# r-barnes/richdem

Measured on NVIDIA H100. Metric: Priority-Flood fill + D8 flow accumulation throughput, higher is better.
Workload: dtype f32

## Files before the change

richdem_b200/csrc/capi.cu:

```cuda
#include "common.cuh"

#include <algorithm>
#include <cstdlib>
#include <type_traits>

namespace rdb {

static thread_local std::string g_last_error;

void capi_set_error(const char *msg) { g_last_error = msg ? msg : "unknown error"; }

Ctx &ctx() {
  static Ctx c;
  return c;
}

static void init_device(int device) {
  Ctx &c = ctx();
  if (c.inited && c.device == device) return;
  if (c.inited) fail("rdb200_init: already initialised on device %d (call rdb200_shutdown first)", c.device);
  int ndev = 0;
  cudaError_t e = cudaGetDeviceCount(&ndev);
  if (e != cudaSuccess || ndev == 0)
    fail("no CUDA device available (%s); librichdem_b200 has no CPU fallback",
// ... 1 lines not shown
  if (device < 0 || device >= ndev) fail("rdb200_init: device %d out of range (0..%d)", device, ndev - 1);
  RDB_CK(cudaSetDevice(device));
  cudaDeviceProp prop;
  RDB_CK(cudaGetDeviceProperties(&prop, device));
  if (prop.major != 9 || prop.minor != 0)
    fail("device %d is sm_%d%d; librichdem_b200 is built for sm_90a (H100) only", device, prop.major,
         prop.minor);
  c.device = device;
  c.num_sms = prop.multiProcessorCount;
  RDB_CK(cudaStreamCreate(&c.own_stream));
  c.stream = c.own_stream;
  RDB_CK(cudaEventCreate(&c.ev0));
  RDB_CK(cudaEventCreate(&c.ev1));
  RDB_CK(cudaEventCreate(&c.evk0));
  RDB_CK(cudaEventCreate(&c.evk1));
  c.pinned_bytes = 1 << 16;
  RDB_CK(cudaMallocHost(&c.pinned, c.pinned_bytes));
  memset(&c.stats, 0, sizeof(c.stats));
  c.inited = true;
}

void ensure_init() {
  Ctx &c = ctx();
  if (c.inited) {
    RDB_CK(cudaSetDevice(c.device));
    return;
  }
  int dev = 0;
  cudaError_t e = cudaGetDevice(&dev);
  if (e != cudaSuccess) dev = 0;
// ... 394 lines not shown
int rdb200_init(int device) {
  return capi_call([&] { init_device(device); });
}

void rdb200_shutdown(void) {
  Ctx &c = ctx();
  if (!c.inited) return;
  cudaSetDevice(c.device);
  cudaStreamSynchronize(c.stream);
  ws_release_all();
  if (c.pinned) cudaFreeHost(c.pinned);
  cudaEventDestroy(c.ev0);
  cudaEventDestroy(c.ev1);
  cudaEventDestroy(c.evk0);
  cudaEventDestroy(c.evk1);
  cudaStreamDestroy(c.own_stream);
  for (int k = 0; k < 2; k++)
    if (c.aux_stream[k]) cudaStreamDestroy(c.aux_stream[k]);
  for (int k = 0; k < 3; k++)
    if (c.aux_event[k]) cudaEventDestroy(c.aux_event[k]);
  const Params keep = c.params;
  c = Ctx();
  c.params = keep;
}

const char *rdb200_last_error(void) { return g_last_error.c_str(); }
int rdb200_version(void) { return RDB200_VERSION; }

int rdb200_set_stream(void *cuda_stream) {
  return capi_call([&] {
// ... 31 lines not shown
    else if (n == "fill_wake_filter") p.fill_wake_filter = value;
    else if (n == "fill_trace") p.fill_trace = value;
    else if (n == "fill_ordered") p.fill_ordered = value;
    else if (n == "fill_order_rounds") p.fill_order_rounds = value;
    else if (n == "fill_band_rounds") p.fill_band_rounds = value;
    else if (n == "accum_threads") p.accum_threads = value > 0 ? value : 256;
    else if (n == "accum_budget") p.accum_budget = value;
    else if (n == "accum_walk_lanes") p.accum_walk_lanes = value;
    else if (n == "accum_fused_prep") p.accum_fused_prep = value;
    else if (n == "flats_tiled") p.flats_tiled = value;
    else if (n == "flats_pair") p.flats_pair = value;
    else if (n == "flats_fused_classify") p.flats_fused_classify = value;
    else if (n == "fill_multigrid") p.fill_multigrid = value;
    else if (n == "fill_multigrid_min") p.fill_multigrid_min = value;
    else if (n == "fill_vcycle") p.fill_vcycle = value;
    else if (n == "fill_band_multigrid") p.fill_band_multigrid = value;
    else if (n == "flats_uf_tiled") p.flats_uf_tiled = value;
    else if (n == "flowdirs_rolling") p.flowdirs_rolling = value;
    else if (n == "accum_packed") p.accum_packed = value;
    else if (n == "accum_dinf_packed") p.accum_dinf_packed = value;
    else if (n == "accum_dinf_share") p.accum_dinf_share = value;
    else if (n == "flowmet_tarboton_filter") p.flowmet_tarboton_filter = value;
    else if (n == "accum_walk_scan") p.accum_walk_scan = value;
    else if (n == "accum_walk_ahead") p.accum_walk_ahead = value;
    else if (n == "accum_dinf_stats") p.accum_dinf_stats = value;
    else if (n == "accum_dinf_wait") p.accum_dinf_wait = value;
    else if (n == "f64_band_rank_cap") p.f64_band_rank_cap = value;
    else fail("rdb200_set_param: unknown parameter '%s'", name);
  });
}
// ... 426 lines not shown
```

richdem_b200/csrc/common.cuh:

```cuda
#pragma once

#include <cuda.h>
#include <cuda_runtime.h>

#include <cstdarg>
#include <cstdint>
#include <cstdio>
#include <cstring>
#include <stdexcept>
#include <string>
#include <vector>

#include "../../include/richdem_b200.h"

struct rdb200_fill_state;

namespace rdb {

struct Error : std::runtime_error {
  using std::runtime_error::runtime_error;
};

[[noreturn]] inline void fail(const char *fmt, ...) {
  char buf[1024];
// ... 34 lines not shown
}

struct Params {
  int64_t fill_max_iters = 0;
  int64_t fill_rounds_per_sync = 16;
  int64_t fill_use_tma = 1;
  int64_t fill_external_z = 1;
  int64_t fill_ordered = 1;
  int64_t fill_order_rounds = 0;
  int64_t fill_band_rounds = 0;
  int64_t fill_profile = 0;
  int64_t fill_wake_filter = 1;
  int64_t fill_trace = 0;
  int64_t fill_multigrid = 8;
  int64_t fill_vcycle = 8;
  int64_t fill_band_multigrid = 0;
  int64_t fill_multigrid_min = 0;
  int64_t flowdirs_rolling = 1;
  int64_t flats_uf_tiled = 1;
  int64_t flats_fused_classify = 1;
  int64_t flats_pair = 1;
  int64_t flats_tiled = 1;
  int64_t accum_dinf_packed = 1;
  int64_t flowmet_tarboton_filter = 1;
  int64_t accum_walk_ahead = 0;
  int64_t accum_walk_scan = 0;
  int64_t accum_dinf_stats = 0;
  int64_t accum_dinf_share = -1;
  int64_t accum_dinf_wait = 0;
  int64_t accum_packed = 1;
// ... 4 lines not shown
  int64_t f64_band_rank_cap = 0;
};

struct WsBlock {
  void *ptr;
  size_t bytes;
  bool in_use;
};

struct Ctx {
  bool inited = false;
  int device = -1;
  int num_sms = 0;
  cudaStream_t stream = nullptr;
  cudaStream_t own_stream = nullptr;
  cudaEvent_t ev0 = nullptr, ev1 = nullptr, evk0 = nullptr, evk1 = nullptr;
  cudaStream_t aux_stream[2] = {nullptr, nullptr};
  cudaEvent_t aux_event[3] = {nullptr, nullptr, nullptr};
  std::vector<WsBlock> ws;
  void *pinned = nullptr;
  size_t pinned_bytes = 0;
  rdb200_stats stats;
  Params params;
};

Ctx &ctx();
void ensure_init();
void *ws_alloc(size_t bytes);
void ws_free(void *p);
void ws_release_all();

// ... 140 lines not shown
```

richdem_b200/csrc/fill.cu:

```cuda
#include "common.cuh"

#include <chrono>
#include <memory>

namespace rdb {

namespace {

#ifndef RDB_TX
#define RDB_TX 64
#endif
#ifndef RDB_TY
#define RDB_TY 64
#endif
#ifndef RDB_FILL_THREADS
#define RDB_FILL_THREADS 128
#endif
#ifndef RDB_FILL_MIN_CTAS
#define RDB_FILL_MIN_CTAS 6
#endif
constexpr int TX = RDB_TX;
constexpr int TY = RDB_TY;
constexpr int BXN = TX / 4;
constexpr int BYN = TY / 4;
// ... 16 lines not shown
  RoundCtl proc[3];
  unsigned long long visits;
  unsigned long long iters;
  unsigned long long block_updates;
  unsigned long long warp_updates;
  unsigned long long idle_visits;
  unsigned long long wakes_dropped;
  unsigned long long iter_hist[8];
  int edge_changed;
  int zmin_ord, zmax_ord;
  unsigned long long deferred;
  unsigned long long live_rounds;
  float level, step, step_min, level_max;
  int target, ordered;
  int ndefer[3];
};

struct FillArgs {
  const float *Z;
  int zpitch, zox, zoy;
  int inplace;
  const float *coarse;
  int Wc, pool, yoff;
  int *staged;
  float *zcopy;
  float *Wp;
  int pitch;
  int wox, woy;
  int W, H;
  int tilesX, tilesY;
  int *list0, *list1;
  int *stamp;
  int *sides;
  int *keys;
  float level;
  int *plist;
  int use_proc;
  FillDev *dev;
  int round;
  int max_iters;
  int use_tma;
  int profile;
  int *dirty;
  unsigned long long *edge_above;
};

__device__ __forceinline__ uint32_t smem_u32(const void *p) {
  return (uint32_t)__cvta_generic_to_shared(p);
}
__device__ __forceinline__ void mbar_init(unsigned long long *bar, int count) {
  asm volatile("mbarrier.init.shared::cta.b64 [%0], %1;" ::"r"(smem_u32(bar)), "r"(count) : "memory");
}
__device__ __forceinline__ void mbar_arrive_expect_tx(unsigned long long *bar, uint32_t bytes) {
  asm volatile("mbarrier.arrive.expect_tx.shared::cta.b64 _, [%0], %1;" ::"r"(smem_u32(bar)),
               "r"(bytes)
               : "memory");
}
__device__ __forceinline__ void mbar_wait(unsigned long long *bar, uint32_t parity) {
// ... 47 lines not shown
  const int b = o >= 0 ? o : (o ^ 0x7fffffff);
  float f;
  memcpy(&f, &b, 4);
  return f;
}
constexpr int ORD_POS_INF = 0x7f800000;

__device__ __forceinline__ void enqueue_tile(const FillArgs &a, RoundCtl *next, int *list_next, int t,
                                             int stampval, int side_bits, int key_ord) {
  atomicOr(&a.sides[(stampval & 1) * a.tilesX * a.tilesY + t], side_bits);
  atomicMin(&a.keys[(stampval & 1) * a.tilesX * a.tilesY + t], key_ord);
  if (atomicExch(&a.stamp[t], stampval) != stampval) {
    const int idx = atomicAdd(&next->count, 1);
    list_next[idx] = t;
  }
}

__device__ __forceinline__ float min3f(float a, float b, float c) { return fminf(fminf(a, b), c); }

__host__ __device__ __forceinline__ float next_up(float x) {
  int b;
  memcpy(&b, &x, 4);
  b = b < 0 ? (b == (int)0x80000000 ? 1 : b - 1) : (b < 0x7f800000 ? b + 1 : b);
  float r;
  memcpy(&r, &b, 4);
  return r;
}

template <int STEP>
__device__ __forceinline__ float fill_step(float w) {
// ... 319 lines not shown
                   *reinterpret_cast<const float4 *>(&sZ[rr * TX + 4 * cc]));
        }
      }
    }
    if (stage) {
      __syncthreads();
      if (tid == 0) {
        __threadfence();
        atomicExch(&a.staged[t], 1);
      }
    }
    if (STEP != 1 && WAKE_WORDS && a.edge_above) {
      fill_wake_neighbours<TOPO4>(a, sW, sZ, t, fl, sKey, next, list_next);
      if (rowch && tid == 0) {
        if (fl & (3 << 9)) atomicOr(&a.dev->edge_changed, (fl >> 9) & 3);
        if (a.dirty) a.dirty[t] = 1;
      }
    } else if (rowch) {
      if (tid < 8) {
        const int sv = r + 1;
        const bool n_ok = tyT > 0, s_ok = tyT < a.tilesY - 1, w_ok = txT > 0, e_ok = txT < a.tilesX - 1;
        int nb = -1, bits = 0;
        switch (tid) {
          case 0: if ((fl & SIDE_N) && n_ok) { nb = t - a.tilesX; bits = SIDE_S; } break;
          case 1: if ((fl & SIDE_S) && s_ok) { nb = t + a.tilesX; bits = SIDE_N; } break;
          case 2: if ((fl & SIDE_W) && w_ok) { nb = t - 1; bits = SIDE_E; } break;
          case 3: if ((fl & SIDE_E) && e_ok) { nb = t + 1; bits = SIDE_W; } break;
          case 4: if ((fl & SIDE_NW) && n_ok && w_ok) { nb = t - a.tilesX - 1; bits = SIDE_SE; } break;
          case 5: if ((fl & SIDE_NE) && n_ok && e_ok) { nb = t - a.tilesX + 1; bits = SIDE_SW; } break;
          case 6: if ((fl & SIDE_SW) && s_ok && w_ok) { nb = t + a.tilesX - 1; bits = SIDE_NE; } break;
          default: if ((fl & SIDE_SE) && s_ok && e_ok) { nb = t + a.tilesX + 1; bits = SIDE_NW; } break;
        }
        if (nb >= 0) enqueue_tile(a, next, list_next, nb, sv, bits, sKey);
        if (tid == 0 && (fl & (3 << 9))) atomicOr(&a.dev->edge_changed, (fl >> 9) & 3);
        if (tid == 0 && a.dirty) a.dirty[t] = 1;
      }
    }
    if (tid == 0) {
      if (again) enqueue_tile(a, next, list_next, t, r + 1, SIDE_FULL, f2ord(-__int_as_float(0x7f800000)));
      atomicAdd(&a.dev->iters, (unsigned long long)iters);
      if (a.profile) {
        if (!rowch) atomicAdd(&a.dev->idle_visits, 1ull);
        atomicAdd(&a.dev->block_updates, (unsigned long long)sProf[0]);
        atomicAdd(&a.dev->warp_updates, (unsigned long long)sProf[1]);
        const int hb = iters <= 1 ? 0 : iters <= 2 ? 1 : iters <= 4 ? 2 : iters <= 8 ? 3 : iters <= 16 ? 4 : iters <= 32 ? 5 : iters <= 64 ? 6 : 7;
        atomicAdd(&a.dev->iter_hist[hb], 1ull);
      }
    }
  }
  if (STAGE && a.use_tma && tid == 0) bulk_wait_all();
// ... 16 lines not shown
    if (ord2f(kord) <= level) {
      a.plist[atomicAdd(&proc->count, 1)] = t;
    } else {
      int bits = a.sides[(r & 1) * ntiles + t];
      if (bits == 0) bits = SIDE_FULL;
      a.sides[(r & 1) * ntiles + t] = 0;
      a.keys[(r & 1) * ntiles + t] = ORD_POS_INF;
      enqueue_tile(a, next, list_next, t, r + 1, bits, kord);
      nd++;
    }
  }
  for (int o = 16; o > 0; o >>= 1) nd += __shfl_xor_sync(0xffffffffu, nd, o);
  if ((threadIdx.x & 31) == 0 && nd) atomicAdd(&a.dev->ndefer[r % 3], nd);
}

__global__ void __launch_bounds__(256) fill_seed_kernel(const FillArgs a, const int *__restrict__ tiles, int n) {
  const int i = blockIdx.x * blockDim.x + threadIdx.x;
  if (i >= n) return;
  const int r = a.round;
  RoundCtl *cur = &a.dev->ctl[r % 3];
  int *list_cur = (r & 1) ? a.list1 : a.list0;
  enqueue_tile(a, cur, list_cur, tiles[i], r, SIDE_FULL, f2ord(-__int_as_float(0x7f800000)));
}

__global__ void __launch_bounds__(256) fill_seed_flags_kernel(const FillArgs a, const int *__restrict__ flag, int ntiles,
                                                               int *count) {
  const int t = blockIdx.x * blockDim.x + threadIdx.x;
  if (t >= ntiles || !flag[t]) return;
  const int r = a.round;
  RoundCtl *cur = &a.dev->ctl[r % 3];
  int *list_cur = (r & 1) ? a.list1 : a.list0;
  enqueue_tile(a, cur, list_cur, t, r, SIDE_FULL, f2ord(-__int_as_float(0x7f800000)));
  if (count) atomicAdd(count, 1);
}

__global__ void __launch_bounds__(256) fill_ghost_update_kernel(float *Wp, float *Zp, int pitch, int W, int H, int y,
                                                                 const float *__restrict__ row, int *tile_flag, int tilesX,
                                                                 int *lowered) {
// ... 189 lines not shown
    }
    float *o = Wc + (size_t)(by + coy) * cpitch + bx + cox;
    if (m < *o && bx > 0 && by > 0 && bx < Wcw - 1 && by < Hc - 1) {
      *o = m;
      const int ty0 = (by - 1) / TY, ty1 = (by + 1) / TY, tx0 = (bx - 1) / TX, tx1 = (bx + 1) / TX;
      ctile_flag[ty0 * ctilesX + tx0] = 1;
      if (tx1 != tx0) ctile_flag[ty0 * ctilesX + tx1] = 1;
      if (ty1 != ty0) {
        ctile_flag[ty1 * ctilesX + tx0] = 1;
        if (tx1 != tx0) ctile_flag[ty1 * ctilesX + tx1] = 1;
      }
    }
  }
}

__global__ void __launch_bounds__(256) fill_blockmax_kernel(const float *__restrict__ Wp, int pitch, int wox, int woy, int W,
                                                             int y_lo, int y_hi,
                                                             int yoff, float *out, int Wcw, int Hc, int k,
                                                             const int *__restrict__ dirty, int tilesX) {
  const int bx = blockIdx.x * blockDim.x + threadIdx.x;
  if (bx >= Wcw) return;
  const int by_lo = (yoff + y_lo) / k, by_hi = (yoff + y_hi - 1) / k;
  for (int by = by_lo + blockIdx.y; by <= by_hi && by < Hc; by += gridDim.y) {
    if (dirty) {
      int l0 = by * k - yoff, l1 = l0 + k - 1;
      l0 = l0 < y_lo ? y_lo : l0;
      l1 = l1 >= y_hi ? y_hi - 1 : l1;
      const int tx = (bx * k) / TX;
      if (!dirty[(l0 / TY) * tilesX + tx] && !dirty[(l1 / TY) * tilesX + tx]) {
        out[(size_t)by * Wcw + bx] = __int_as_float(0x7f800000);
// ... 3 lines not shown
    float m = -__int_as_float(0x7f800000);
    for (int j = 0; j < k; j++) {
      const int y = by * k + j - yoff;
      if (y < y_lo) continue;
      if (y >= y_hi) break;
      for (int i = 0; i < k; i++) {
        const int x = bx * k + i;
        if (x < W) m = fmaxf(m, __ldcg(Wp + (size_t)(y + woy) * pitch + x + wox));
      }
    }
    float *o = out + (size_t)by * Wcw + bx;
    *o = fmaxf(*o, m);
  }
}

__global__ void __launch_bounds__(256) fill_prolong_kernel(float *Wp, int pitch, int wox, int woy, int W, int H,
                                                            const float *__restrict__ Wc,
                                                            int cpitch, int coff_x, int coff_y, int k, int *tile_flag,
                                                            int tilesX, int yoff, const int *__restrict__ cdirty,
                                                            int ctilesX) {
  const int t = blockIdx.x;
  const int tyT = t / tilesX, txT = t - tyT * tilesX;
  const int x0 = txT * TX, y0 = tyT * TY;
  if (cdirty) {
    const int cx0 = (x0 / k) / TX, cx1 = ((x0 + TX - 1) / k) / TX;
    const int cy0 = ((y0 + yoff) / k) / TY, cy1 = ((y0 + TY - 1 + yoff) / k) / TY;
    bool any = false;
    for (int cy = cy0; cy <= cy1; cy++)
      for (int cx = cx0; cx <= cx1; cx++) any |= cdirty[cy * ctilesX + cx] != 0;
    if (!any) return;
  }
  bool lowered = false, lo_n = false, lo_s = false, lo_w = false, lo_e = false;
  for (int g = threadIdx.x; g < TX * TY / 4; g += blockDim.x) {
    const int ly = g / (TX / 4), lx4 = (g - ly * (TX / 4)) * 4;
    const int y = y0 + ly;
    if (y < 1 || y >= H - 1 || x0 + lx4 >= W) continue;
    float4 *wp4 = reinterpret_cast<float4 *>(Wp + (size_t)(y + woy) * pitch + x0 + lx4 + wox);
    const float4 w4 = *wp4;
    float wv[4] = {w4.x, w4.y, w4.z, w4.w};
    const float *crow = Wc + (size_t)((y + yoff) / k + coff_y) * cpitch + coff_x;
    bool any = false;
#pragma unroll
    for (int j = 0; j < 4; j++) {
      const int lx = lx4 + j, x = x0 + lx;
      if (x < 1 || x >= W - 1) continue;
      const float l = __ldg(crow + x / k);
      if (l < wv[j]) {
        wv[j] = l;
        any = true;
        lo_w |= lx == 0;
        lo_e |= lx == TX - 1;
      }
    }
    if (any) {
      *wp4 = make_float4(wv[0], wv[1], wv[2], wv[3]);
      lowered = true;
      lo_n |= ly == 0;
      lo_s |= ly == TY - 1;
    }
  }
  if (lowered) {
    const int tilesY = (H + TY - 1) / TY;
    tile_flag[t] = 1;
    const bool n_ok = tyT > 0, s_ok = tyT < tilesY - 1, w_ok = txT > 0, e_ok = txT < tilesX - 1;
    if (lo_n && n_ok) tile_flag[t - tilesX] = 1;
    if (lo_s && s_ok) tile_flag[t + tilesX] = 1;
    if (lo_w && w_ok) tile_flag[t - 1] = 1;
    if (lo_e && e_ok) tile_flag[t + 1] = 1;
    if (lo_n && lo_w && n_ok && w_ok) tile_flag[t - tilesX - 1] = 1;
    if (lo_n && lo_e && n_ok && e_ok) tile_flag[t - tilesX + 1] = 1;
    if (lo_s && lo_w && s_ok && w_ok) tile_flag[t + tilesX - 1] = 1;
    if (lo_s && lo_e && s_ok && e_ok) tile_flag[t + tilesX + 1] = 1;
  }
}

__global__ void __launch_bounds__(256) fill_finish_x4_kernel(const float *__restrict__ Wp, float *__restrict__ out, int W,
                                                              int H, int pitch, int wox, int woy) {
  const int x4 = (blockIdx.x * blockDim.x + threadIdx.x) * 4;
  if (x4 >= W) return;
  for (int y = blockIdx.y; y < H; y += gridDim.y) {
    const float4 v = __ldcs(reinterpret_cast<const float4 *>(Wp + (size_t)(y + woy) * pitch + x4 + wox));
    __stcs(reinterpret_cast<float4 *>(out + (size_t)y * W + x4), v);
  }
}

__global__ void fill_finish_kernel(const float *__restrict__ Wp, float *__restrict__ out, int W, int H,
                                   int pitch, int wox, int woy) {
// ... 27 lines not shown
  const cuuint32_t estr[2] = {1, 1};
  CUresult rc = get_encode_fn()(&m, CU_TENSOR_MAP_DATA_TYPE_FLOAT32, 2, base, gdim, gstride, box, estr,
                                CU_TENSOR_MAP_INTERLEAVE_NONE, CU_TENSOR_MAP_SWIZZLE_NONE,
                                CU_TENSOR_MAP_L2_PROMOTION_L2_128B, CU_TENSOR_MAP_FLOAT_OOB_FILL_NONE);
  if (rc != CUDA_SUCCESS) fail("cuTensorMapEncodeTiled failed with CUresult %d", (int)rc);
  return m;
}

}

struct FillState {
  int W = 0, H = 0, pitch = 0, rows = 0, tilesX = 0, tilesY = 0;
  DevBuf<float> Zp, Wp;
  DevBuf<int> list0, list1, plist, stamp, sides, keys;
  DevBuf<int> dirty, tflag;
  DevBuf<int> staged;
  DevBuf<unsigned long long> edge_above;
  float zmin = 0.f, zmax = 0.f;
  bool first_run = true;
  bool ordered = false;
  int step_mode = 0;
  bool topo4 = false;
  float pin = __builtin_nanf("");
  std::vector<float> levels;
  DevBuf<FillDev> dev;
  CUtensorMap mapW, mapZ;
  int round = 0;
  int grid = 0;
  int64_t rounds_run = 0;
  int64_t live_rounds = 0;
// ... 54 lines not shown
    keys.alloc(2 * nt);
    dev.alloc(1);
    RDB_CK(cudaMemsetAsync(stamp.p, 0, nt * sizeof(int), c.stream));
    RDB_CK(cudaMemsetAsync(sides.p, 0, 2 * nt * sizeof(int), c.stream));
    if (stage_coarse) {
      staged.alloc(nt);
      RDB_CK(cudaMemsetAsync(staged.p, 0, nt * sizeof(int), c.stream));
    }
    edge_above.alloc(4 * nt);
    RDB_CK(cudaMemsetAsync(edge_above.p, 0xff, 4 * nt * sizeof(unsigned long long), c.stream));
    {
      FillDev h0;
      memset(&h0, 0, sizeof(h0));
      h0.zmin_ord = ORD_POS_INF;
      h0.zmax_ord = f2ord(-__builtin_inff());
      memcpy(c.pinned, &h0, sizeof(h0));
      RDB_CK(cudaMemcpyAsync(dev.p, c.pinned, sizeof(FillDev), cudaMemcpyHostToDevice, c.stream));
    }
    {
      const int n2 = (int)(2 * nt);
      fill_i32_kernel<<<(n2 + 255) / 256, 256, 0, c.stream>>>(keys.p, ORD_POS_INF, n2);
      count_launch();
      dim3 blk(128), grd((pitch / 4 + 127) / 128, rows < 2048 ? rows : 2048);
      if (stage_coarse) {
      } else if (inplace) {
        dim3 grdc((W / 4 + 127) / 128, H < 2048 ? H : 2048);
        fill_init_kernel<false><<<grdc, blk, 0, c.stream>>>(d_dem, Zc.p, Wb, W, H, W, H, 0, 0, dev.p, nullptr, 0, 1, 0, pin);
        count_launch();
      } else if (d_coarse) {
        fill_init_kernel<true><<<grd, blk, 0, c.stream>>>(d_dem, Zp.p, Wp.p, W, H, pitch, rows, PADL, 1, dev.p, d_coarse,
                                                         coarse_w, coarse_k, coarse_yoff, pin);
        count_launch();
// ... 49 lines not shown
    }
    if (inplace) {
      mapW = make_map(Wb, W, H, SP, SROWS);
      mapZ = make_map(Zc.p, W, H, TX, TY);
      if (stage_coarse) mapZstage = make_map(Wb, W, H, TX, TY);
    } else {
      mapW = make_map(Wp.p, pitch, rows, SP, SROWS);
      mapZ = make_map(Zp.p, pitch, rows, TX, TY);
    }
    int per_sm = 0;
    RDB_CK(cudaOccupancyMaxActiveBlocksPerMultiprocessor(
        &per_sm, step_mode == 2 ? (const void *)fill_sweep_kernel<2> : (const void *)fill_sweep_kernel<0>, FILL_THREADS, 0));
    if (per_sm < 1) per_sm = 1;
    grid = c.num_sms * per_sm;
    round = 1;
    std::vector<int> init;
    for (int ty = 0; ty < tilesY; ty++)
      for (int tx = 0; tx < tilesX; tx++)
        if (d_coarse || step_mode == 2 || ty == 0 || tx == 0 || ty == tilesY - 1 || tx == tilesX - 1)
          init.push_back(ty * tilesX + tx);
    seed_worklist(init);
  }

  void begin_dist(const uint8_t *d_open, int open_bit, const float *d_winit, int w, int h, int ghost_top = 0,
                  int ghost_bottom = 0) {
    Ctx &c = ctx();
    step_mode = 1;
    W = w;
    H = h;
    tilesX = (w + TX - 1) / TX;
    tilesY = (h + TY - 1) / TY;
    pitch = tilesX * TX + 2 * PADL;
    rows = tilesY * TY + 2;
    use_padded_layout((size_t)pitch * rows);
    const size_t nt = (size_t)tilesX * tilesY;
// ... 65 lines not shown
    a.H = H;
    a.tilesX = tilesX;
    a.tilesY = tilesY;
    a.list0 = list0.p;
    a.list1 = list1.p;
    a.stamp = stamp.p;
    a.sides = sides.p;
    a.keys = keys.p;
    a.plist = plist.p;
    a.dev = dev.p;
    a.max_iters = (int)c.params.fill_max_iters;
    a.use_tma = (int)c.params.fill_use_tma;
    a.profile = (int)c.params.fill_profile;
    a.level = __builtin_inff();
    a.dirty = dirty.p;
    a.edge_above = step_mode != 1 && c.params.fill_wake_filter != 0 ? edge_above.p : nullptr;
    return a;
  }

  bool timed = true;
  int batch_edge = 0;
  void launch_batch(int per_sync) {
    Ctx &c = ctx();
    FillArgs a = make_args();
    if (timed) RDB_CK(cudaEventRecord(c.evk0, c.stream));
    for (int k = 0; k < per_sync; k++) {
      a.round = round;
      if (ordered && sched_round < (int64_t)levels.size()) {
        a.level = levels[(size_t)sched_round];
        a.use_proc = 1;
        fill_admit_kernel<<<c.num_sms * 2, 256, 0, c.stream>>>(a);
        c.stats.kernel_launches++;
      } else {
        a.level = __builtin_inff();
        a.use_proc = 0;
      }
      sched_round++;
      a.coarse = round == 1 ? stage_coarse : nullptr;
      a.Z = a.coarse ? Wb : (inplace ? Zc.p : Zp.p);
      a.zcopy = a.coarse ? Zc.p : nullptr;
      const CUtensorMap &mz = a.coarse ? mapZstage : mapZ;
      if (step_mode == 1) fill_sweep_kernel<1><<<grid, FILL_THREADS, 0, c.stream>>>(mapW, mz, mapZ, a);
      else if (step_mode == 2 && topo4) fill_sweep_kernel<2, true><<<grid, FILL_THREADS, 0, c.stream>>>(mapW, mz, mapZ, a);
      else if (step_mode == 2) fill_sweep_kernel<2><<<grid, FILL_THREADS, 0, c.stream>>>(mapW, mz, mapZ, a);
      else if (a.coarse && topo4) fill_sweep_kernel<0, true, true><<<grid, FILL_THREADS, 0, c.stream>>>(mapW, mz, mapZ, a);
      else if (a.coarse) fill_sweep_kernel<0, false, true><<<grid, FILL_THREADS, 0, c.stream>>>(mapW, mz, mapZ, a);
      else if (topo4) fill_sweep_kernel<0, true><<<grid, FILL_THREADS, 0, c.stream>>>(mapW, mz, mapZ, a);
      else fill_sweep_kernel<0><<<grid, FILL_THREADS, 0, c.stream>>>(mapW, mz, mapZ, a);
      round++;
    }
    if (timed) RDB_CK(cudaEventRecord(c.evk1, c.stream));
    RDB_CK(cudaGetLastError());
    RDB_CK(cudaMemcpyAsync(c.pinned, dev.p, sizeof(FillDev), cudaMemcpyDeviceToHost, c.stream));
    c.stats.kernel_launches += per_sync;
    rounds_run += per_sync;
    if (round > (1 << 30)) fail("fill: round counter overflow");
  }
  bool collect() {
    Ctx &c = ctx();
    RDB_CK(cudaStreamSynchronize(c.stream));
    if (timed) {
      float t = 0;
      RDB_CK(cudaEventElapsedTime(&t, c.evk0, c.evk1));
      c.stats.ms_main_kernel += t;
    }
    const FillDev *hd = (const FillDev *)c.pinned;
    still_active = hd->ctl[round % 3].count != 0;
    if (!still_active) first_run = false;
    live_rounds = (int64_t)hd->live_rounds;
    visits_seen = (int64_t)hd->visits;
    iters_seen = (int64_t)hd->iters;
    batch_edge = hd->edge_changed;
    return still_active;
  }
  int64_t iters_seen = 0;

  int run(int64_t max_rounds = 0) {
    Ctx &c = ctx();
    int64_t rounds_this_call = 0;
    int per_sync = (int)(c.params.fill_rounds_per_sync > 0 ? c.params.fill_rounds_per_sync : 16);
    if (max_rounds > 0 && max_rounds < per_sync) per_sync = (int)max_rounds;
    RDB_CK(cudaMemsetAsync(&dev.p->edge_changed, 0, sizeof(int), c.stream));
    for (;;) {
      launch_batch(per_sync);
      collect();
      rounds_this_call += per_sync;
      if (!still_active) break;
      if (max_rounds > 0 && rounds_this_call >= max_rounds) break;
    }
    const FillDev *hd = (const FillDev *)c.pinned;
    c.stats.fill_rounds = live_rounds;
    c.stats.fill_tile_visits = visits_seen;
    c.stats.fill_tile_iters = iters_seen;
    c.stats.fill_tile_cells = TX * TY;
    if (c.params.fill_profile) {
      fprintf(stderr, "[fill profile] deferred=%llu visits=%llu iters=%llu block_updates=%llu (%.1f%% of 256/iter) warp_updates=%llu (%.1f%% of 8/iter) idle_visits=%llu wakes_dropped=%llu hist(1,2,3-4,5-8,9-16,17-32,33-64,65+)=",
              hd->deferred, hd->visits, hd->iters, hd->block_updates, 100.0 * hd->block_updates / (256.0 * hd->iters + 1),
              hd->warp_updates, 100.0 * hd->warp_updates / (8.0 * hd->iters + 1), hd->idle_visits, hd->wakes_dropped);
      for (int k = 0; k < 8; k++) fprintf(stderr, "%llu ", hd->iter_hist[k]);
      fprintf(stderr, "\n");
      fprintf(stderr, "[fill wake] visits=%llu idle_visits=%llu wakes_dropped=%llu\n", hd->visits - prof_seen[0],
              hd->idle_visits - prof_seen[1], hd->wakes_dropped - prof_seen[2]);
      prof_seen[0] = hd->visits;
      prof_seen[1] = hd->idle_visits;
      prof_seen[2] = hd->wakes_dropped;
    }
    return batch_edge | (still_active ? 4 : 0);
  }
  unsigned long long prof_seen[3] = {0, 0, 0};

  void track_dirty() {
    Ctx &c = ctx();
    const size_t nt = (size_t)tilesX * tilesY;
    dirty.alloc(nt);
    RDB_CK(cudaMemsetAsync(dirty.p, 0, nt * sizeof(int), c.stream));
  }
  void clear_dirty() {
    if (dirty.p) RDB_CK(cudaMemsetAsync(dirty.p, 0, (size_t)tilesX * tilesY * sizeof(int), ctx().stream));
  }
  void seed_from_flags(int *d_count = nullptr) {
    Ctx &c = ctx();
    const int nt = tilesX * tilesY;
    FillArgs a = make_args();
    a.round = round;
    fill_seed_flags_kernel<<<(nt + 255) / 256, 256, 0, c.stream>>>(a, tflag.p, nt, d_count);
    RDB_CK(cudaGetLastError());
    count_launch();
  }
  void clear_flags() {
    const size_t nt = (size_t)tilesX * tilesY;
    if (!tflag.p) tflag.alloc(nt);
    RDB_CK(cudaMemsetAsync(tflag.p, 0, nt * sizeof(int), ctx().stream));
  }
  void restrict_into(FillState &cs, int k) {
    Ctx &c = ctx();
    cs.clear_flags();
    const bool selective = dirty.p && TX % k == 0 && TY % k == 0;
    dim3 blk(256), grd((unsigned)((cs.W + 255) / 256), (unsigned)(cs.H < 4096 ? cs.H : 4096));
    fill_restrict_kernel<<<grd, blk, 0, c.stream>>>(Wb, wpitch, wox, woy, W, H, cs.Wb, cs.wpitch, cs.wox, cs.woy, cs.W, cs.H,
                                                    k, selective ? dirty.p : nullptr, tilesX, cs.tflag.p, cs.tilesX);
    RDB_CK(cudaGetLastError());
    count_launch();
    cs.seed_from_flags();
    clear_dirty();
  }
  void blockmax_into(float *d_out, int wc, int hc, int k, int yoff, int y_lo, int y_hi, bool selective = false) {
    Ctx &c = ctx();
    dim3 blk(256), grd((unsigned)((wc + 255) / 256), (unsigned)((y_hi - y_lo) / k + 2 < 4096 ? (y_hi - y_lo) / k + 2 : 4096));
    const bool sel = selective && dirty.p && TX % k == 0;
    fill_blockmax_kernel<<<grd, blk, 0, c.stream>>>(Wb, wpitch, wox, woy, W, y_lo, y_hi, yoff, d_out, wc, hc, k,
                                                    sel ? dirty.p : nullptr, tilesX);
    RDB_CK(cudaGetLastError());
    count_launch();
    if (sel) clear_dirty();
  }
  void prolong_from(const float *d_wc, int cpitch, int coff_x, int coff_y, int k, int yoff = 0, const int *cdirty = nullptr,
                    int ctilesX = 0, int *d_count = nullptr) {
    Ctx &c = ctx();
    clear_flags();
    const int nt = tilesX * tilesY;
    fill_prolong_kernel<<<nt, 256, 0, c.stream>>>(Wb, wpitch, wox, woy, W, H, d_wc, cpitch, coff_x, coff_y, k, tflag.p, tilesX,
                                                  yoff, cdirty, ctilesX);
    RDB_CK(cudaGetLastError());
    count_launch();
    seed_from_flags(d_count);
  }
  void prolong_from_level(FillState &cs, int k, int yoff = 0, int *d_count = nullptr) {
    prolong_from(cs.Wb, cs.wpitch, cs.wox, cs.woy, k, yoff, cs.dirty.p, cs.tilesX, d_count);
    cs.clear_dirty();
  }
  void ghost_update(int y, const float *d_row, int *d_lowered) {
    Ctx &c = ctx();
    clear_flags();
    fill_ghost_update_kernel<<<(W + 255) / 256, 256, 0, c.stream>>>(Wp.p, Zp.p, pitch, W, H, y, d_row, tflag.p, tilesX, d_lowered);
    RDB_CK(cudaGetLastError());
    count_launch();
    seed_from_flags();
  }

  void read_row(int y, float *d_row) {
    if (y < 0 || y >= H) fail("fill_read_row: row %d out of range", y);
    RDB_CK(cudaMemcpyAsync(d_row, Wb + (size_t)(y + woy) * wpitch + wox, (size_t)W * 4,
// ... 144 lines not shown
      zc.alloc((size_t)wc * hc);
      RDB_CK(cudaMemcpyAsync(zc.p, coarse.p, (size_t)wc * hc * sizeof(float), cudaMemcpyDeviceToDevice, c.stream));
    }
    const rdb200_stats before = c.stats;
    fill_depressions_level(coarse.p, wc, hc, depth + 1, topo4);
    rdb200_stats extra = c.stats;
    extra.fill_rounds -= before.fill_rounds;
    extra.fill_tile_visits -= before.fill_tile_visits;
    extra.fill_tile_iters -= before.fill_tile_iters;
    st.begin(d_dem, w, h, coarse.p, wc, k, 0, true);
    if (every <= 0) {
      st.run();
    } else {
      FillState cst;
      cst.topo4 = topo4;
      cst.begin(zc.p, wc, hc, coarse.p, wc, 1, 0, true);
      cst.run();
      cst.track_dirty();
      st.track_dirty();
      int64_t coarse_visits0 = c.stats.fill_tile_visits, coarse_iters0 = c.stats.fill_tile_iters;
      const bool trace = c.params.fill_trace != 0;
      auto now_ms = [&]() {
        RDB_CK(cudaStreamSynchronize(c.stream));
        return std::chrono::duration<double, std::milli>(std::chrono::steady_clock::now().time_since_epoch()).count();
      };
      for (int cycle = 0;; cycle++) {
        const double t0 = trace ? now_ms() : 0;
        const int64_t v0 = st.visits_seen, r0 = st.live_rounds;
        const bool active = (st.run(every) & 4) != 0;
        const double t1 = trace ? now_ms() : 0;
        if (trace)
          fprintf(stderr, "[fill trace] depth %d cycle %d: fine run %.3f ms (%lld live rounds, %lld visits)%s\n", depth, cycle,
                  t1 - t0, (long long)(st.live_rounds - r0), (long long)(st.visits_seen - v0), active ? "" : " -> converged");
        if (!active) break;
        if (cycle >= 1000) {
          st.run();
          break;
        }
        st.restrict_into(cst, k);
        const double t2 = trace ? now_ms() : 0;
        const int64_t cv0 = cst.visits_seen, cr0 = cst.live_rounds;
        cst.run();
        const double t3 = trace ? now_ms() : 0;
        st.prolong_from_level(cst, k);
        if (trace) {
          const double t4 = now_ms();
          fprintf(stderr, "[fill trace] depth %d cycle %d: restrict %.3f ms, coarse run %.3f ms (%lld live rounds, %lld visits), "
                          "prolong %.3f ms\n", depth, cycle, t2 - t1, t3 - t2, (long long)(cst.live_rounds - cr0),
                  (long long)(cst.visits_seen - cv0), t4 - t3);
        }
      }
      cst.run(1);
      extra.fill_rounds += cst.live_rounds;
      extra.fill_tile_visits += c.stats.fill_tile_visits;
      extra.fill_tile_iters += c.stats.fill_tile_iters;
      (void)coarse_visits0;
      (void)coarse_iters0;
      st.run(1);
    }
    st.finish(d_dem);
    RDB_CK(cudaStreamSynchronize(c.stream));
    c.stats.fill_rounds = st.live_rounds + extra.fill_rounds;
    c.stats.fill_tile_visits += extra.fill_tile_visits;
    c.stats.fill_tile_iters += extra.fill_tile_iters;
    return;
  }
  if (w <= 2 || h <= 2) return;
  st.begin(d_dem, w, h, nullptr, 0, 0, 0, true);
  st.run();
  st.finish(d_dem);
  RDB_CK(cudaStreamSynchronize(c.stream));
}

// ... 353 lines not shown
```

Baseline: 22170.

## Pipeline V-cycle fill with list-driven restrict/prolong and fewer host syncs

```diff
diff --git a/richdem_b200/csrc/capi.cu b/richdem_b200/csrc/capi.cu
--- a/richdem_b200/csrc/capi.cu
+++ b/richdem_b200/csrc/capi.cu
@@ -39,6 +39,8 @@
   RDB_CK(cudaEventCreate(&c.ev1));
   RDB_CK(cudaEventCreate(&c.evk0));
   RDB_CK(cudaEventCreate(&c.evk1));
+  RDB_CK(cudaEventCreate(&c.evk2));
+  RDB_CK(cudaEventCreate(&c.evk3));
   c.pinned_bytes = 1 << 16;
   RDB_CK(cudaMallocHost(&c.pinned, c.pinned_bytes));
   memset(&c.stats, 0, sizeof(c.stats));
@@ -463,6 +465,8 @@
   cudaEventDestroy(c.ev1);
   cudaEventDestroy(c.evk0);
   cudaEventDestroy(c.evk1);
+  cudaEventDestroy(c.evk2);
+  cudaEventDestroy(c.evk3);
   cudaStreamDestroy(c.own_stream);
   for (int k = 0; k < 2; k++)
     if (c.aux_stream[k]) cudaStreamDestroy(c.aux_stream[k]);
@@ -524,6 +528,7 @@
     else if (n == "fill_multigrid") p.fill_multigrid = value;
     else if (n == "fill_multigrid_min") p.fill_multigrid_min = value;
     else if (n == "fill_vcycle") p.fill_vcycle = value;
+    else if (n == "fill_vcycle_coarse") p.fill_vcycle_coarse = value > 0 ? value : 16;
     else if (n == "fill_band_multigrid") p.fill_band_multigrid = value;
     else if (n == "flats_uf_tiled") p.flats_uf_tiled = value;
     else if (n == "flowdirs_rolling") p.flowdirs_rolling = value;
diff --git a/richdem_b200/csrc/common.cuh b/richdem_b200/csrc/common.cuh
--- a/richdem_b200/csrc/common.cuh
+++ b/richdem_b200/csrc/common.cuh
@@ -72,6 +72,7 @@
   int64_t fill_trace = 0;
   int64_t fill_multigrid = 8;
   int64_t fill_vcycle = 8;
+  int64_t fill_vcycle_coarse = 16;
   int64_t fill_band_multigrid = 0;
   int64_t fill_multigrid_min = 0;
   int64_t flowdirs_rolling = 1;
@@ -106,7 +107,7 @@
   int num_sms = 0;
   cudaStream_t stream = nullptr;
   cudaStream_t own_stream = nullptr;
-  cudaEvent_t ev0 = nullptr, ev1 = nullptr, evk0 = nullptr, evk1 = nullptr;
+  cudaEvent_t ev0 = nullptr, ev1 = nullptr, evk0 = nullptr, evk1 = nullptr, evk2 = nullptr, evk3 = nullptr;
   cudaStream_t aux_stream[2] = {nullptr, nullptr};
   cudaEvent_t aux_event[3] = {nullptr, nullptr, nullptr};
   std::vector<WsBlock> ws;
diff --git a/richdem_b200/csrc/fill.cu b/richdem_b200/csrc/fill.cu
--- a/richdem_b200/csrc/fill.cu
+++ b/richdem_b200/csrc/fill.cu
@@ -54,6 +54,7 @@
   float level, step, step_min, level_max;
   int target, ordered;
   int ndefer[3];
+  int dirty_count;
 };
 
 struct FillArgs {
@@ -82,6 +83,7 @@
   int use_tma;
   int profile;
   int *dirty;
+  int *dirty_list;
   unsigned long long *edge_above;
 };
 
@@ -159,6 +161,10 @@
     const int idx = atomicAdd(&next->count, 1);
     list_next[idx] = t;
   }
+}
+
+__device__ __forceinline__ void mark_written(const FillArgs &a, int t) {
+  if (atomicExch(&a.dirty[t], 1) == 0) a.dirty_list[atomicAdd(&a.dev->dirty_count, 1)] = t;
 }
 
 __device__ __forceinline__ float min3f(float a, float b, float c) { return fminf(fminf(a, b), c); }
@@ -508,7 +514,7 @@
       fill_wake_neighbours<TOPO4>(a, sW, sZ, t, fl, sKey, next, list_next);
       if (rowch && tid == 0) {
         if (fl & (3 << 9)) atomicOr(&a.dev->edge_changed, (fl >> 9) & 3);
-        if (a.dirty) a.dirty[t] = 1;
+        if (a.dirty) mark_written(a, t);
       }
     } else if (rowch) {
       if (tid < 8) {
@@ -527,7 +533,7 @@
         }
         if (nb >= 0) enqueue_tile(a, next, list_next, nb, sv, bits, sKey);
         if (tid == 0 && (fl & (3 << 9))) atomicOr(&a.dev->edge_changed, (fl >> 9) & 3);
-        if (tid == 0 && a.dirty) a.dirty[t] = 1;
+        if (tid == 0 && a.dirty) mark_written(a, t);
       }
     }
     if (tid == 0) {
@@ -574,6 +580,11 @@
   if ((threadIdx.x & 31) == 0 && nd) atomicAdd(&a.dev->ndefer[r % 3], nd);
 }
 
+__device__ __forceinline__ void seed_tile(const FillArgs &a, int t) {
+  const int r = a.round;
+  enqueue_tile(a, &a.dev->ctl[r % 3], (r & 1) ? a.list1 : a.list0, t, r, SIDE_FULL, f2ord(-__int_as_float(0x7f800000)));
+}
+
 __global__ void __launch_bounds__(256) fill_seed_kernel(const FillArgs a, const int *__restrict__ tiles, int n) {
   const int i = blockIdx.x * blockDim.x + threadIdx.x;
   if (i >= n) return;
@@ -582,6 +593,13 @@
   int *list_cur = (r & 1) ? a.list1 : a.list0;
   enqueue_tile(a, cur, list_cur, tiles[i], r, SIDE_FULL, f2ord(-__int_as_float(0x7f800000)));
 }
+
+__global__ void __launch_bounds__(256) fill_seed_all_kernel(const FillArgs a, int ntiles) {
+  const int t = blockIdx.x * blockDim.x + threadIdx.x;
+  if (t < ntiles) seed_tile(a, t);
+}
+
+__global__ void fill_dev_init_kernel(FillDev *dev, const FillDev h0) { *dev = h0; }
 
 __global__ void __launch_bounds__(256) fill_seed_flags_kernel(const FillArgs a, const int *__restrict__ flag, int ntiles,
                                                                int *count) {
@@ -801,6 +819,57 @@
   }
 }
 
+__global__ void __launch_bounds__(256) fill_restrict_list_kernel(const float *__restrict__ Wp, int pitch, int wox, int woy,
+                                                                  int W, int H, float *Wc, int cpitch, int cox, int coy,
+                                                                  int Wcw, int Hc, int k, int *dirty,
+                                                                  const int *__restrict__ list, const int *count, int tilesX,
+                                                                  int *ctile_flag, int ctilesX) {
+  const int cw = TX / k, cells = cw * (TY / k);
+  const long long items = (long long)*count * cells;
+  for (long long it = blockIdx.x * (long long)blockDim.x + threadIdx.x; it < items; it += (long long)gridDim.x * blockDim.x) {
+    const int li = (int)(it / cells), cell = (int)(it - (long long)li * cells);
+    const int t = list[li];
+    const int tyT = t / tilesX, txT = t - tyT * tilesX;
+    const int bx = txT * cw + cell % cw, by = tyT * (TY / k) + cell / cw;
+    if (cell == 0) dirty[t] = 0;
+    if (bx >= Wcw || by >= Hc) continue;
+    float m = -__int_as_float(0x7f800000);
+    const float *blk = Wp + (size_t)(by * k + woy) * pitch + bx * k + wox;
+    if (k == 8 && bx * k + k <= W && by * k + k <= H) {
+      float4 q[16];
+#pragma unroll
+      for (int j = 0; j < 8; j++) {
+        q[2 * j] = __ldcg(reinterpret_cast<const float4 *>(blk + (size_t)j * pitch));
+        q[2 * j + 1] = __ldcg(reinterpret_cast<const float4 *>(blk + (size_t)j * pitch) + 1);
+      }
+#pragma unroll
+      for (int j = 0; j < 16; j++) m = fmaxf(fmaxf(m, fmaxf(q[j].x, q[j].y)), fmaxf(q[j].z, q[j].w));
+    } else if ((k & 3) == 0 && bx * k + k <= W && by * k + k <= H) {
+      for (int j = 0; j < k; j++) {
+        const float4 *row = reinterpret_cast<const float4 *>(blk + (size_t)j * pitch);
+        for (int i = 0; i < k / 4; i++) {
+          const float4 q = __ldcg(row + i);
+          m = fmaxf(fmaxf(m, fmaxf(q.x, q.y)), fmaxf(q.z, q.w));
+        }
+      }
+    } else {
+      for (int j = 0; j < k && by * k + j < H; j++)
+        for (int i = 0; i < k && bx * k + i < W; i++) m = fmaxf(m, __ldcg(blk + (size_t)j * pitch + i));
+    }
+    float *o = Wc + (size_t)(by + coy) * cpitch + bx + cox;
+    if (m < *o && bx > 0 && by > 0 && bx < Wcw - 1 && by < Hc - 1) {
+      *o = m;
+      const int ty0 = (by - 1) / TY, ty1 = (by + 1) / TY, tx0 = (bx - 1) / TX, tx1 = (bx + 1) / TX;
+      ctile_flag[ty0 * ctilesX + tx0] = 1;
+      if (tx1 != tx0) ctile_flag[ty0 * ctilesX + tx1] = 1;
+      if (ty1 != ty0) {
+        ctile_flag[ty1 * ctilesX + tx0] = 1;
+        if (tx1 != tx0) ctile_flag[ty1 * ctilesX + tx1] = 1;
+      }
+    }
+  }
+}
+
 __global__ void __launch_bounds__(256) fill_blockmax_kernel(const float *__restrict__ Wp, int pitch, int wox, int woy, int W,
                                                              int y_lo, int y_hi,
                                                              int yoff, float *out, int Wcw, int Hc, int k,
@@ -834,22 +903,8 @@
   }
 }
 
-__global__ void __launch_bounds__(256) fill_prolong_kernel(float *Wp, int pitch, int wox, int woy, int W, int H,
-                                                            const float *__restrict__ Wc,
-                                                            int cpitch, int coff_x, int coff_y, int k, int *tile_flag,
-                                                            int tilesX, int yoff, const int *__restrict__ cdirty,
-                                                            int ctilesX) {
-  const int t = blockIdx.x;
-  const int tyT = t / tilesX, txT = t - tyT * tilesX;
-  const int x0 = txT * TX, y0 = tyT * TY;
-  if (cdirty) {
-    const int cx0 = (x0 / k) / TX, cx1 = ((x0 + TX - 1) / k) / TX;
-    const int cy0 = ((y0 + yoff) / k) / TY, cy1 = ((y0 + TY - 1 + yoff) / k) / TY;
-    bool any = false;
-    for (int cy = cy0; cy <= cy1; cy++)
-      for (int cx = cx0; cx <= cx1; cx++) any |= cdirty[cy * ctilesX + cx] != 0;
-    if (!any) return;
-  }
+__device__ __forceinline__ int prolong_tile(float *Wp, int pitch, int wox, int woy, int W, int H, const float *__restrict__ Wc,
+                                            int cpitch, int coff_x, int coff_y, int k, int yoff, int x0, int y0) {
   bool lowered = false, lo_n = false, lo_s = false, lo_w = false, lo_e = false;
   for (int g = threadIdx.x; g < TX * TY / 4; g += blockDim.x) {
     const int ly = g / (TX / 4), lx4 = (g - ly * (TX / 4)) * 4;
@@ -879,10 +934,32 @@
       lo_s |= ly == TY - 1;
     }
   }
-  if (lowered) {
+  if (!lowered) return 0;
+  return (lo_n ? SIDE_N : 0) | (lo_s ? SIDE_S : 0) | (lo_w ? SIDE_W : 0) | (lo_e ? SIDE_E : 0) | SIDE_FULL;
+}
+
+__global__ void __launch_bounds__(256) fill_prolong_kernel(float *Wp, int pitch, int wox, int woy, int W, int H,
+                                                            const float *__restrict__ Wc,
+                                                            int cpitch, int coff_x, int coff_y, int k, int *tile_flag,
+                                                            int tilesX, int yoff, const int *__restrict__ cdirty,
+                                                            int ctilesX) {
+  const int t = blockIdx.x;
+  const int tyT = t / tilesX, txT = t - tyT * tilesX;
+  const int x0 = txT * TX, y0 = tyT * TY;
+  if (cdirty) {
+    const int cx0 = (x0 / k) / TX, cx1 = ((x0 + TX - 1) / k) / TX;
+    const int cy0 = ((y0 + yoff) / k) / TY, cy1 = ((y0 + TY - 1 + yoff) / k) / TY;
+    bool any = false;
+    for (int cy = cy0; cy <= cy1; cy++)
+      for (int cx = cx0; cx <= cx1; cx++) any |= cdirty[cy * ctilesX + cx] != 0;
+    if (!any) return;
+  }
+  const int lo = prolong_tile(Wp, pitch, wox, woy, W, H, Wc, cpitch, coff_x, coff_y, k, yoff, x0, y0);
+  if (lo) {
     const int tilesY = (H + TY - 1) / TY;
     tile_flag[t] = 1;
     const bool n_ok = tyT > 0, s_ok = tyT < tilesY - 1, w_ok = txT > 0, e_ok = txT < tilesX - 1;
+    const bool lo_n = lo & SIDE_N, lo_s = lo & SIDE_S, lo_w = lo & SIDE_W, lo_e = lo & SIDE_E;
     if (lo_n && n_ok) tile_flag[t - tilesX] = 1;
     if (lo_s && s_ok) tile_flag[t + tilesX] = 1;
     if (lo_w && w_ok) tile_flag[t - 1] = 1;
@@ -891,6 +968,48 @@
     if (lo_n && lo_e && n_ok && e_ok) tile_flag[t - tilesX + 1] = 1;
     if (lo_s && lo_w && s_ok && w_ok) tile_flag[t + tilesX - 1] = 1;
     if (lo_s && lo_e && s_ok && e_ok) tile_flag[t + tilesX + 1] = 1;
+  }
+}
+
+__global__ void __launch_bounds__(256) fill_prolong_list_kernel(const FillArgs a, const float *__restrict__ Wc, int cpitch,
+                                                                 int coff_x, int coff_y, int k, int *cdirty,
+                                                                 const int *__restrict__ clist, const int *ccount,
+                                                                 int ctilesX, const float *__restrict__ Ws, int cW, int cH) {
+  __shared__ int sLo;
+  const int per = k * k;
+  const int items = *ccount * per;
+  for (int item = blockIdx.x; item < items; item += gridDim.x) {
+    const int li = item / per, s = item - li * per;
+    const int ct = clist[li];
+    const int cty = ct / ctilesX, ctx = ct - cty * ctilesX;
+    const int tyT = cty * k + s / k, txT = ctx * k + s % k;
+    if (s == 0 && threadIdx.x == 0) cdirty[ct] = 0;
+    if (tyT >= a.tilesY || txT >= a.tilesX) continue;
+    if (Ws) {
+      const int cw = TX / k, cells = cw * (TY / k);
+      bool moved = false;
+      for (int i = threadIdx.x; i < cells; i += blockDim.x) {
+        const int bx = txT * cw + i % cw, by = tyT * (TY / k) + i / cw;
+        if (bx < cW && by < cH) {
+          const size_t o = (size_t)(by + coff_y) * cpitch + bx + coff_x;
+          moved |= !(Wc[o] >= Ws[o]);
+        }
+      }
+      if (!__syncthreads_or(moved)) continue;
+    }
+    if (threadIdx.x == 0) sLo = 0;
+    __syncthreads();
+    const int lo = prolong_tile(a.Wp, a.pitch, a.wox, a.woy, a.W, a.H, Wc, cpitch, coff_x, coff_y, k, 0, txT * TX, tyT * TY);
+    if (lo) atomicOr(&sLo, lo);
+    __syncthreads();
+    const int l = sLo;
+    if (l && threadIdx.x < 9) {
+      const int dy = threadIdx.x / 3 - 1, dx = threadIdx.x % 3 - 1;
+      const bool rows_ok = dy == 0 || (dy < 0 ? (l & SIDE_N) && tyT > 0 : (l & SIDE_S) && tyT < a.tilesY - 1);
+      const bool cols_ok = dx == 0 || (dx < 0 ? (l & SIDE_W) && txT > 0 : (l & SIDE_E) && txT < a.tilesX - 1);
+      if (rows_ok && cols_ok) seed_tile(a, (tyT + dy) * a.tilesX + txT + dx);
+    }
+    __syncthreads();
   }
 }
 
@@ -948,6 +1067,7 @@
   DevBuf<float> Zp, Wp;
   DevBuf<int> list0, list1, plist, stamp, sides, keys;
   DevBuf<int> dirty, tflag;
+  DevBuf<int> dirty_list;
   DevBuf<int> staged;
   DevBuf<unsigned long long> edge_above;
   float zmin = 0.f, zmax = 0.f;
@@ -1032,8 +1152,8 @@
       memset(&h0, 0, sizeof(h0));
       h0.zmin_ord = ORD_POS_INF;
       h0.zmax_ord = f2ord(-__builtin_inff());
-      memcpy(c.pinned, &h0, sizeof(h0));
-      RDB_CK(cudaMemcpyAsync(dev.p, c.pinned, sizeof(FillDev), cudaMemcpyHostToDevice, c.stream));
+      fill_dev_init_kernel<<<1, 1, 0, c.stream>>>(dev.p, h0);
+      count_launch();
     }
     {
       const int n2 = (int)(2 * nt);
@@ -1113,11 +1233,18 @@
     if (per_sm < 1) per_sm = 1;
     grid = c.num_sms * per_sm;
     round = 1;
+    if (d_coarse || step_mode == 2) {
+      FillArgs a = make_args();
+      a.round = round;
+      fill_seed_all_kernel<<<(unsigned)((nt + 255) / 256), 256, 0, c.stream>>>(a, (int)nt);
+      RDB_CK(cudaGetLastError());
+      count_launch();
+      return;
+    }
     std::vector<int> init;
     for (int ty = 0; ty < tilesY; ty++)
       for (int tx = 0; tx < tilesX; tx++)
-        if (d_coarse || step_mode == 2 || ty == 0 || tx == 0 || ty == tilesY - 1 || tx == tilesX - 1)
-          init.push_back(ty * tilesX + tx);
+        if (ty == 0 || tx == 0 || ty == tilesY - 1 || tx == tilesX - 1) init.push_back(ty * tilesX + tx);
     seed_worklist(init);
   }
 
@@ -1213,16 +1340,20 @@
     a.profile = (int)c.params.fill_profile;
     a.level = __builtin_inff();
     a.dirty = dirty.p;
+    a.dirty_list = dirty_list.p;
     a.edge_above = step_mode != 1 && c.params.fill_wake_filter != 0 ? edge_above.p : nullptr;
     return a;
   }
 
   bool timed = true;
+  bool second = false;
   int batch_edge = 0;
+  static constexpr size_t SECOND_SLOT = 3 * 8192;
+  FillDev *readback() { return (FillDev *)((char *)ctx().pinned + (second ? SECOND_SLOT : 0)); }
   void launch_batch(int per_sync) {
     Ctx &c = ctx();
     FillArgs a = make_args();
-    if (timed) RDB_CK(cudaEventRecord(c.evk0, c.stream));
+    if (timed) RDB_CK(cudaEventRecord(second ? c.evk2 : c.evk0, c.stream));
     for (int k = 0; k < per_sync; k++) {
       a.round = round;
       if (ordered && sched_round < (int64_t)levels.size()) {
@@ -1248,22 +1379,25 @@
       else fill_sweep_kernel<0><<<grid, FILL_THREADS, 0, c.stream>>>(mapW, mz, mapZ, a);
       round++;
     }
-    if (timed) RDB_CK(cudaEventRecord(c.evk1, c.stream));
+    if (timed) RDB_CK(cudaEventRecord(second ? c.evk3 : c.evk1, c.stream));
     RDB_CK(cudaGetLastError());
-    RDB_CK(cudaMemcpyAsync(c.pinned, dev.p, sizeof(FillDev), cudaMemcpyDeviceToHost, c.stream));
+    RDB_CK(cudaMemcpyAsync(readback(), dev.p, sizeof(FillDev), cudaMemcpyDeviceToHost, c.stream));
     c.stats.kernel_launches += per_sync;
     rounds_run += per_sync;
     if (round > (1 << 30)) fail("fill: round counter overflow");
   }
   bool collect() {
+    RDB_CK(cudaStreamSynchronize(ctx().stream));
+    return take();
+  }
+  bool take() {
     Ctx &c = ctx();
-    RDB_CK(cudaStreamSynchronize(c.stream));
     if (timed) {
       float t = 0;
-      RDB_CK(cudaEventElapsedTime(&t, c.evk0, c.evk1));
+      RDB_CK(cudaEventElapsedTime(&t, second ? c.evk2 : c.evk0, second ? c.evk3 : c.evk1));
       c.stats.ms_main_kernel += t;
     }
-    const FillDev *hd = (const FillDev *)c.pinned;
+    const FillDev *hd = readback();
     still_active = hd->ctl[round % 3].count != 0;
     if (!still_active) first_run = false;
     live_rounds = (int64_t)hd->live_rounds;
@@ -1287,7 +1421,7 @@
       if (!still_active) break;
       if (max_rounds > 0 && rounds_this_call >= max_rounds) break;
     }
-    const FillDev *hd = (const FillDev *)c.pinned;
+    const FillDev *hd = readback();
     c.stats.fill_rounds = live_rounds;
     c.stats.fill_tile_visits = visits_seen;
     c.stats.fill_tile_iters = iters_seen;
@@ -1312,10 +1446,14 @@
     Ctx &c = ctx();
     const size_t nt = (size_t)tilesX * tilesY;
     dirty.alloc(nt);
+    dirty_list.alloc(nt);
     RDB_CK(cudaMemsetAsync(dirty.p, 0, nt * sizeof(int), c.stream));
+    RDB_CK(cudaMemsetAsync(&dev.p->dirty_count, 0, sizeof(int), c.stream));
   }
   void clear_dirty() {
-    if (dirty.p) RDB_CK(cudaMemsetAsync(dirty.p, 0, (size_t)tilesX * tilesY * sizeof(int), ctx().stream));
+    if (!dirty.p) return;
+    RDB_CK(cudaMemsetAsync(dirty.p, 0, (size_t)tilesX * tilesY * sizeof(int), ctx().stream));
+    RDB_CK(cudaMemsetAsync(&dev.p->dirty_count, 0, sizeof(int), ctx().stream));
   }
   void seed_from_flags(int *d_count = nullptr) {
     Ctx &c = ctx();
@@ -1335,13 +1473,22 @@
     Ctx &c = ctx();
     cs.clear_flags();
     const bool selective = dirty.p && TX % k == 0 && TY % k == 0;
-    dim3 blk(256), grd((unsigned)((cs.W + 255) / 256), (unsigned)(cs.H < 4096 ? cs.H : 4096));
-    fill_restrict_kernel<<<grd, blk, 0, c.stream>>>(Wb, wpitch, wox, woy, W, H, cs.Wb, cs.wpitch, cs.wox, cs.woy, cs.W, cs.H,
-                                                    k, selective ? dirty.p : nullptr, tilesX, cs.tflag.p, cs.tilesX);
-    RDB_CK(cudaGetLastError());
-    count_launch();
+    if (selective) {
+      fill_restrict_list_kernel<<<c.num_sms * 8, 256, 0, c.stream>>>(Wb, wpitch, wox, woy, W, H, cs.Wb, cs.wpitch, cs.wox,
+                                                                     cs.woy, cs.W, cs.H, k, dirty.p, dirty_list.p,
+                                                                     &dev.p->dirty_count, tilesX, cs.tflag.p, cs.tilesX);
+      RDB_CK(cudaGetLastError());
+      count_launch();
+      RDB_CK(cudaMemsetAsync(&dev.p->dirty_count, 0, sizeof(int), c.stream));
+    } else {
+      dim3 blk(256), grd((unsigned)((cs.W + 255) / 256), (unsigned)(cs.H < 4096 ? cs.H : 4096));
+      fill_restrict_kernel<<<grd, blk, 0, c.stream>>>(Wb, wpitch, wox, woy, W, H, cs.Wb, cs.wpitch, cs.wox, cs.woy, cs.W, cs.H,
+                                                      k, selective ? dirty.p : nullptr, tilesX, cs.tflag.p, cs.tilesX);
+      RDB_CK(cudaGetLastError());
+      count_launch();
+      clear_dirty();
+    }
     cs.seed_from_flags();
-    clear_dirty();
   }
   void blockmax_into(float *d_out, int wc, int hc, int k, int yoff, int y_lo, int y_hi, bool selective = false) {
     Ctx &c = ctx();
@@ -1364,7 +1511,19 @@
     count_launch();
     seed_from_flags(d_count);
   }
-  void prolong_from_level(FillState &cs, int k, int yoff = 0, int *d_count = nullptr) {
+  void prolong_from_level(FillState &cs, int k, int yoff = 0, int *d_count = nullptr, const float *snap = nullptr) {
+    Ctx &c = ctx();
+    if (cs.dirty_list.p && yoff == 0 && !d_count && TX % k == 0 && TY % k == 0) {
+      FillArgs a = make_args();
+      a.round = round;
+      fill_prolong_list_kernel<<<c.num_sms * 8, 256, 0, c.stream>>>(a, cs.Wb, cs.wpitch, cs.wox, cs.woy, k, cs.dirty.p,
+                                                                    cs.dirty_list.p, &cs.dev.p->dirty_count, cs.tilesX,
+                                                                    snap, cs.W, cs.H);
+      RDB_CK(cudaGetLastError());
+      count_launch();
+      RDB_CK(cudaMemsetAsync(&cs.dev.p->dirty_count, 0, sizeof(int), c.stream));
+      return;
+    }
     prolong_from(cs.Wb, cs.wpitch, cs.wox, cs.woy, k, yoff, cs.dirty.p, cs.tilesX, d_count);
     cs.clear_dirty();
   }
@@ -1539,11 +1698,14 @@
     } else {
       FillState cst;
       cst.topo4 = topo4;
+      cst.second = true;
       cst.begin(zc.p, wc, hc, coarse.p, wc, 1, 0, true);
       cst.run();
       cst.track_dirty();
       st.track_dirty();
-      int64_t coarse_visits0 = c.stats.fill_tile_visits, coarse_iters0 = c.stats.fill_tile_iters;
+      const int budget = (int)c.params.fill_vcycle_coarse;
+      const size_t snap_n = cst.inplace ? (size_t)cst.W * cst.H : (size_t)cst.pitch * cst.rows;
+      DevBuf<float> snap(snap_n);
       const bool trace = c.params.fill_trace != 0;
       auto now_ms = [&]() {
         RDB_CK(cudaStreamSynchronize(c.stream));
@@ -1551,37 +1713,41 @@
       };
       for (int cycle = 0;; cycle++) {
         const double t0 = trace ? now_ms() : 0;
-        const int64_t v0 = st.visits_seen, r0 = st.live_rounds;
-        const bool active = (st.run(every) & 4) != 0;
+        const int64_t v0 = st.visits_seen, r0 = st.live_rounds, cv0 = cst.visits_seen, cr0 = cst.live_rounds;
+        st.launch_batch(every);
         const double t1 = trace ? now_ms() : 0;
+        st.restrict_into(cst, k);
+        RDB_CK(cudaMemcpyAsync(snap.p, cst.Wb, snap_n * sizeof(float), cudaMemcpyDeviceToDevice, c.stream));
+        const double t2 = trace ? now_ms() : 0;
+        cst.launch_batch(budget);
+        const double t3 = trace ? now_ms() : 0;
+        st.prolong_from_level(cst, k, 0, nullptr, snap.p);
+        RDB_CK(cudaStreamSynchronize(c.stream));
+        const double t4 = trace ? now_ms() : 0;
+        const bool active = st.take();
+        cst.take();
+        while (active && cst.still_active) {
+          cst.launch_batch(budget);
+          st.prolong_from_level(cst, k, 0, nullptr, snap.p);
+          cst.collect();
+        }
         if (trace)
-          fprintf(stderr, "[fill trace] depth %d cycle %d: fine run %.3f ms (%lld live rounds, %lld visits)%s\n", depth, cycle,
-                  t1 - t0, (long long)(st.live_rounds - r0), (long long)(st.visits_seen - v0), active ? "" : " -> converged");
+          fprintf(stderr, "[fill trace] depth %d cycle %d: fine run %.3f ms (%lld live rounds, %lld visits)%s, restrict %.3f ms, "
+                          "coarse run %.3f ms (%lld live rounds, %lld visits%s), prolong %.3f ms\n", depth, cycle, t1 - t0,
+                  (long long)(st.live_rounds - r0), (long long)(st.visits_seen - v0), active ? "" : " -> converged", t2 - t1,
+                  t3 - t2, (long long)(cst.live_rounds - cr0), (long long)(cst.visits_seen - cv0),
+                  cst.still_active ? ", work left" : "", t4 - t3);
         if (!active) break;
         if (cycle >= 1000) {
           st.run();
           break;
         }
-        st.restrict_into(cst, k);
-        const double t2 = trace ? now_ms() : 0;
-        const int64_t cv0 = cst.visits_seen, cr0 = cst.live_rounds;
-        cst.run();
-        const double t3 = trace ? now_ms() : 0;
-        st.prolong_from_level(cst, k);
-        if (trace) {
-          const double t4 = now_ms();
-          fprintf(stderr, "[fill trace] depth %d cycle %d: restrict %.3f ms, coarse run %.3f ms (%lld live rounds, %lld visits), "
-                          "prolong %.3f ms\n", depth, cycle, t2 - t1, t3 - t2, (long long)(cst.live_rounds - cr0),
-                  (long long)(cst.visits_seen - cv0), t4 - t3);
-        }
-      }
-      cst.run(1);
+      }
+      if (cst.run(1) & 4) cst.run();
       extra.fill_rounds += cst.live_rounds;
       extra.fill_tile_visits += c.stats.fill_tile_visits;
       extra.fill_tile_iters += c.stats.fill_tile_iters;
-      (void)coarse_visits0;
-      (void)coarse_iters0;
-      st.run(1);
+      if (st.run(1) & 4) st.run();
     }
     st.finish(d_dem);
     RDB_CK(cudaStreamSynchronize(c.stream));
```

New measurement: 22560 (median of 6 runs). 1.02x the previous value.
